# MayDomine/Burst-Attention

Measured on AMD Instinct MI355X. Metric: attention_fwd_TFLOPs_per_GPU, higher is better.
Workload: dtype fp16; 1 GPU; b=1 seq=262144 h=32 d=128 non-causal; parallelism=ring sequence parallel, sp1

## Files before the change

### burst_attn_amd/build_ext.py

```python

import os
import subprocess
import sys
import sysconfig

PKG_DIR = os.path.dirname(os.path.abspath(__file__))
CSRC = os.path.join(PKG_DIR, "csrc")
BUILD = os.path.join(PKG_DIR, "csrc", "_build")
ARCH = os.environ.get("PYTORCH_ROCM_ARCH", "gfx950")
HIPCC = os.environ.get("HIPCC", "/opt/rocm/bin/hipcc")

DEVICE_SOURCES = ["attn_fwd.hip", "attn_bwd.hip", "probes.hip"]
HOST_SOURCES = ["ext_torch.cpp"]


def _run(cmd, verbose):
    if verbose:
        print("+ " + " ".join(cmd), flush=True)
    r = subprocess.run(cmd, capture_output=True, text=True)
    if r.returncode != 0:
        sys.stderr.write(r.stdout + r.stderr)
        raise RuntimeError(f"build command failed: {' '.join(cmd[:3])} ...")
    return r


def _newer(src, dst):
    return not os.path.exists(dst) or os.path.getmtime(src) > os.path.getmtime(dst)


def build(verbose=True, force=False):
    import torch
    from torch.utils import cpp_extension

    os.makedirs(BUILD, exist_ok=True)
    out_so = os.path.join(PKG_DIR, "_C.so")

    torch_includes = cpp_extension.include_paths()
    py_include = sysconfig.get_paths()["include"]
    abi = int(torch._C._GLIBCXX_USE_CXX11_ABI)

    common = [
        f"--offload-arch={ARCH}", "-O3", "-std=c++17", "-fPIC",
        "-DNDEBUG",
    ]
    objs = []
    abihdr = os.path.join(PKG_DIR, "..", "include", "burst_attn_hip.h")
    hdrs = [abihdr] + [os.path.join(CSRC, h) for h in sorted(os.listdir(CSRC))
                       if h.endswith(".h")]
    for src in DEVICE_SOURCES:
        sp = os.path.join(CSRC, src)
        op = os.path.join(BUILD, src.replace(".hip", ".o"))
        objs.append(op)
        if force or _newer(sp, op) or any(_newer(h, op) for h in hdrs):
            _run([HIPCC, *common, "-c", sp, "-o", op], verbose)
    for src in HOST_SOURCES:
        sp = os.path.join(CSRC, src)
        op = os.path.join(BUILD, src.replace(".cpp", ".o"))
        objs.append(op)
        if force or _newer(sp, op) or any(_newer(h, op) for h in hdrs):
            cmd = [
                HIPCC, *common,
                f"-D_GLIBCXX_USE_CXX11_ABI={abi}",
                "-DTORCH_EXTENSION_NAME=_C",
                "-DTORCH_API_INCLUDE_EXTENSION_H",
                "-DUSE_ROCM=1", "-D__HIP_PLATFORM_AMD__=1",
            ]
            for inc in torch_includes + [py_include]:
                cmd += ["-I", inc]
            cmd += ["-c", sp, "-o", op]
            _run(cmd, verbose)
    if force or any(_newer(o, out_so) for o in objs):
        lib_dirs = cpp_extension.library_paths()
        cmd = [HIPCC, "-shared", "-fPIC", *objs, "-o", out_so]
        for ld in lib_dirs:
            cmd += [f"-L{ld}", f"-Wl,-rpath,{ld}"]
        cmd += ["-ltorch", "-ltorch_cpu", "-ltorch_python", "-lc10",
                "-ltorch_hip", "-lc10_hip", "-lamdhip64"]
        _run(cmd, verbose)
    _build_asm_hsaco(verbose, force)
    if verbose:
        print(f"built {out_so}")
    return out_so


LLVM = os.path.join(os.path.dirname(os.path.dirname(HIPCC)), "lib", "llvm",
                    "bin") if "rocm" in HIPCC else "/opt/rocm/lib/llvm/bin"


def _build_asm_hsaco(verbose, force):
    import json
    import re

    src = os.path.join(CSRC, "attn_fwd.hip")
    s_path = os.path.join(BUILD, "attn_fwd_scaffold.s")
    o_path = os.path.join(BUILD, "attn_fwd_scaffold.o")
    hsaco = os.path.join(PKG_DIR, "_asm_fwd.hsaco")
    syms = os.path.join(PKG_DIR, "_asm_fwd_syms.json")
    patch_mod = os.path.join(PKG_DIR, "..", "tools", "s_patch.py")
    if not (force or _newer(src, hsaco) or _newer(patch_mod, hsaco)):
        return hsaco
    _run([HIPCC, f"--offload-arch={ARCH}", "-O3", "-std=c++17", "-DNDEBUG",
          "-S", "--cuda-device-only", src, "-o", s_path], verbose)
    clang = os.path.join(LLVM, "clang")
    lld = os.path.join(LLVM, "ld.lld")
    _run([clang, "-x", "assembler", "-target", "amdgcn-amd-amdhsa",
          f"-mcpu={ARCH}", "-c", s_path, "-o", o_path], verbose)
    _run([lld, "-shared", o_path, "-o", hsaco], verbose)
    text = open(s_path).read()
    names = {}
    for key, pat in (
        ("f16_accum", r"_ZN12_GLOBAL__N_115attn_fwd_kernelIDF16_Li128ELi64ELi1ELi0ELi1ELi512ELi2ELi0ELi0EJEE\S*"),
        ("bf16_accum", r"_ZN12_GLOBAL__N_115attn_fwd_kernelIDF16bLi128ELi64ELi1ELi0ELi1ELi512ELi2ELi0ELi0EJEE\S*"),
    ):
        m = re.search(r"\.globl\t(" + pat + ")", text)
        if m:
            names[key] = m.group(1)
    with open(syms, "w") as f:
        json.dump(names, f, indent=1)
    import importlib.util

    spec = importlib.util.spec_from_file_location("s_patch", patch_mod)
    s_patch = importlib.util.module_from_spec(spec)
    spec.loader.exec_module(s_patch)
    sp_path = os.path.join(BUILD, "attn_fwd_patched.s")
    spo_path = os.path.join(BUILD, "attn_fwd_patched.o")
    hsaco_p = os.path.join(PKG_DIR, "_asm_fwd_p.hsaco")
    s_patch.apply("qk_split", s_path, sp_path, list(names.values()))
    _run([clang, "-x", "assembler", "-target", "amdgcn-amd-amdhsa",
          f"-mcpu={ARCH}", "-c", sp_path, "-o", spo_path], verbose)
    _run([lld, "-shared", spo_path, "-o", hsaco_p], verbose)
    if verbose:
        print(f"built {hsaco} and {hsaco_p} (qk_split)")
    return hsaco


if __name__ == "__main__":
    build(force="--force" in sys.argv)
```

### burst_attn_amd/csrc/attn_common.h

```cpp
#pragma once
#include <hip/hip_runtime.h>
#include <stdint.h>

#include "band_support.h"

typedef __attribute__((ext_vector_type(8))) __bf16 bf16x8_t;
typedef __attribute__((ext_vector_type(8))) _Float16 f16x8_t;
typedef __attribute__((ext_vector_type(16))) float f32x16_t;
typedef __attribute__((ext_vector_type(2))) int i32x2_t;
typedef __attribute__((ext_vector_type(4))) unsigned int u32x4_t;

__device__ __forceinline__ float ba_exp2(float x) {
  return __builtin_amdgcn_exp2f(x);
}

#define BA_LOG2E 1.44269504088896340736f
#define BA_LN2 0.69314718055994530942f
#define BA_NEG_BIG (-1e30f)

template <typename T>
struct mfma_traits;

template <>
struct mfma_traits<_Float16> {
  using frag = f16x8_t;
  static __device__ __forceinline__ f32x16_t mma(frag a, frag b, f32x16_t c) {
    return __builtin_amdgcn_mfma_f32_32x32x16_f16(a, b, c, 0, 0, 0);
  }
  static __device__ __forceinline__ unsigned int bits(float x) {
    _Float16 h = (_Float16)x;
    return (unsigned int)__builtin_bit_cast(unsigned short, h);
  }
  static __device__ __forceinline__ unsigned int pack2(float lo, float hi) {
    return __builtin_bit_cast(unsigned int, __builtin_amdgcn_cvt_pkrtz(lo, hi));
  }
};

template <>
struct mfma_traits<__bf16> {
  using frag = bf16x8_t;
  static __device__ __forceinline__ f32x16_t mma(frag a, frag b, f32x16_t c) {
    return __builtin_amdgcn_mfma_f32_32x32x16_bf16(a, b, c, 0, 0, 0);
  }
  static __device__ __forceinline__ unsigned int bits(float x) {
    __bf16 h = (__bf16)x;
    return (unsigned int)__builtin_bit_cast(unsigned short, h);
  }
  static __device__ __forceinline__ unsigned int pack2(float lo, float hi) {
    return bits(lo) | (bits(hi) << 16);
  }
};

__device__ __forceinline__ constexpr int ba_crow(int r, int hi) {
  return (r & 3) + 8 * (r >> 2) + 4 * hi;
}

template <int SWZ, int SWZ2 = 0>
__device__ __forceinline__ int ba_swz(int byte, int row) {
  return byte ^ ((((row & SWZ) ^ ((row >> 3) & SWZ2))) << 4);
}

template <typename T>
__device__ __forceinline__ void ba_build_frag_pair(
    const f32x16_t& p, typename mfma_traits<T>::frag out[2]) {
  using MT = mfma_traits<T>;
#pragma unroll
  for (int u = 0; u < 2; ++u) {
    unsigned int a0 = MT::pack2(p[8 * u + 0], p[8 * u + 1]);
    unsigned int a1 = MT::pack2(p[8 * u + 2], p[8 * u + 3]);
    unsigned int b0 = MT::pack2(p[8 * u + 4], p[8 * u + 5]);
    unsigned int b1 = MT::pack2(p[8 * u + 6], p[8 * u + 7]);
    i32x2_t r0 = __builtin_amdgcn_permlane32_swap((int)a0, (int)b0, false, false);
    i32x2_t r1 = __builtin_amdgcn_permlane32_swap((int)a1, (int)b1, false, false);
    u32x4_t w = {(unsigned int)r0[0], (unsigned int)r1[0],
                 (unsigned int)r0[1], (unsigned int)r1[1]};
    out[u] = __builtin_bit_cast(typename mfma_traits<T>::frag, w);
  }
}

__device__ __forceinline__ void ba_half_pair(float x, float& lo, float& hi) {
  const int xi = __builtin_bit_cast(int, x);
  const i32x2_t r = __builtin_amdgcn_permlane32_swap(xi, xi, false, false);
  lo = __builtin_bit_cast(float, (int)r[0]);
  hi = __builtin_bit_cast(float, (int)r[1]);
}

struct ba_seg_args {
  const int32_t* q_seg;
  const int32_t* kv_seg;
  int64_t q_sb, kv_sb;
  const int2* tile_mm;
  const int2* blk_range;
};
__device__ __forceinline__ ba_seg_args ba_seg_of() { return {}; }
__device__ __forceinline__ ba_seg_args ba_seg_of(const ba_seg_args& s) {
  return s;
}

template <typename A, typename B>
struct ba_same_t {
  static constexpr bool value = false;
};
template <typename A>
struct ba_same_t<A, A> {
  static constexpr bool value = true;
};
template <typename A, typename... P>
constexpr bool ba_pack_is = sizeof...(P) == 1 && (ba_same_t<A, P>::value && ...);
__device__ __forceinline__ ba_band_args ba_band_of(const ba_band_args& b) {
  return b;
}

__device__ __forceinline__ void ba_wave_minmax(int x, int& mn, int& mx) {
  mn = mx = x;
#pragma unroll
  for (int o = 32; o; o >>= 1) {
    mn = min(mn, __shfl_xor(mn, o));
    mx = max(mx, __shfl_xor(mx, o));
  }
  mn = __builtin_amdgcn_readfirstlane(mn);
  mx = __builtin_amdgcn_readfirstlane(mx);
}

__device__ __forceinline__ float ba_max16(const f32x16_t& v) {
  float a = fmaxf(fmaxf(v[0], v[1]), v[2]);
  float b = fmaxf(fmaxf(v[3], v[4]), v[5]);
  float c = fmaxf(fmaxf(v[6], v[7]), v[8]);
  float d = fmaxf(fmaxf(v[9], v[10]), v[11]);
  float e = fmaxf(fmaxf(v[12], v[13]), v[14]);
  float f = fmaxf(fmaxf(a, b), v[15]);
  return fmaxf(fmaxf(fmaxf(c, d), e), f);
}

template <typename T, int RS, int SWZ, int SWZ2 = 0>
__device__ __forceinline__ typename mfma_traits<T>::frag ba_ld_rowslice(
    const T* lds, int row, int elem0) {
  int byte = ba_swz<SWZ, SWZ2>(row * (2 * RS) + 2 * elem0, row);
  u32x4_t wv = *(const u32x4_t*)((const char*)lds + byte);
  return __builtin_bit_cast(typename mfma_traits<T>::frag, wv);
}

template <typename T, int RS_T, int SWZ_T, int SWZ2_T = 7>
__device__ __forceinline__ void ba_st_transposed(T* lds, int src_row, int d0,
                                                 const u32x4_t& chunk) {
  const T* e = (const T*)&chunk;
#pragma unroll
  for (int j = 0; j < 8; ++j) {
    const int row = d0 + j;
    const int byte = ba_swz<SWZ_T, SWZ2_T>(row * (2 * RS_T) + 2 * src_row, row);
    *(T*)((char*)lds + byte) = e[j];
  }
}

typedef __attribute__((ext_vector_type(4))) short s16x4_t;
typedef __attribute__((ext_vector_type(2))) unsigned int u32x2_t;

template <typename T, int D>
__device__ __forceinline__ int ba_tr16_byte(int lane, int kv0, int dbase) {
  const int kvr = kv0 + 8 * (lane >> 5) + ((lane >> 2) & 3);
  const int e16 = kvr * D + dbase + 16 * ((lane >> 4) & 1) + 4 * (lane & 3);
  return (2 * e16) ^ ((kvr & 7) << 3);
}

template <typename T, int D>
__device__ __forceinline__ typename mfma_traits<T>::frag ba_ld_tr16_frag(
    const T* lds, int lane, int kv0, int dbase) {
  auto p0 = (__attribute__((address_space(3))) s16x4_t*)((
      __attribute__((address_space(3))) char*)(lds) +
      ba_tr16_byte<T, D>(lane, kv0, dbase));
  auto p1 = (__attribute__((address_space(3))) s16x4_t*)((
      __attribute__((address_space(3))) char*)(lds) +
      ba_tr16_byte<T, D>(lane, kv0 + 4, dbase));
  s16x4_t lo = __builtin_amdgcn_ds_read_tr16_b64_v4i16(p0);
  s16x4_t hi = __builtin_amdgcn_ds_read_tr16_b64_v4i16(p1);
  u32x2_t l2 = __builtin_bit_cast(u32x2_t, lo);
  u32x2_t h2 = __builtin_bit_cast(u32x2_t, hi);
  u32x4_t w = {l2[0], l2[1], h2[0], h2[1]};
  return __builtin_bit_cast(typename mfma_traits<T>::frag, w);
}

template <typename T, int D>
__device__ __forceinline__ void ba_st_tr16row(T* lds, int kv, int d0,
                                              const u32x4_t& chunk) {
  const int b0 = (2 * (kv * D + d0)) ^ ((kv & 7) << 3);
  const int b1 = (2 * (kv * D + d0 + 4)) ^ ((kv & 7) << 3);
  u32x2_t lohalf = {chunk.x, chunk.y};
  u32x2_t hihalf = {chunk.z, chunk.w};
  *(u32x2_t*)((char*)lds + b0) = lohalf;
  *(u32x2_t*)((char*)lds + b1) = hihalf;
}
```

### burst_attn_amd/csrc/attn_fwd.hip

```cpp

#include "attn_common.h"
#include "attn_host.h"
#include "fwd_variants.h"
#include "gqa_heads.h"
#include "seg_support.h"
#include "vt_image.h"

#include <stddef.h>

namespace {

template <int N>
struct ba_ic {
  static constexpr int value = N;
};
struct ba_dyn {
  int value;
};
template <int N>
__device__ __forceinline__ int ba_buf_of(ba_ic<N>) { return N; }
__device__ __forceinline__ int ba_buf_of(ba_dyn d) { return d.value; }

template <typename T, int D, int KVBLK, int OUT_STATE, int VPATH, int SUBT,
          int NT = 512, int NBUF = 2, int KREG = 0, int VSRC = 0,
          typename... SEG>
__global__ __launch_bounds__(NT) void attn_fwd_kernel(
    const T* __restrict__ q, const T* __restrict__ k, const T* __restrict__ v,
    float* __restrict__ o, float* __restrict__ lse,
    int Sq, int Sk, int N, int G,
    int64_t q_sb, int64_t q_ss, int64_t q_sh,
    int64_t k_sb, int64_t k_ss, int64_t k_sh,
    int64_t v_sb, int64_t v_ss, int64_t v_sh,
    float scale, int causal,
    float* __restrict__ st_acc, float* __restrict__ st_m,
    float* __restrict__ st_l,
    int64_t a_sb, int64_t a_ss, int64_t a_sh,
    int64_t ml_sb, int64_t ml_sh, int carry_in, SEG... seg) {
  using MT = mfma_traits<T>;
  using frag = typename MT::frag;
  constexpr bool HAS_BAND = ba_pack_is<ba_band_args, SEG...>;
  constexpr bool HAS_SEG = sizeof...(SEG) != 0 && !HAS_BAND;
  constexpr bool HAS_MASK = HAS_SEG || HAS_BAND;
  static_assert(!HAS_MASK || (sizeof...(SEG) == 1 && VPATH == 0 && SUBT == 1 &&
                              NT == 512 && NBUF == 2 && KREG == 0 && VSRC == 0),
                "segment ids / band: the default variant, V transposed "
                "in-kernel");
  static_assert(!HAS_BAND || (KVBLK == BA_BAND_TILE && NT / 2 == BA_BAND_BLOCK),
                "band: the tile sizes of band_support.h");
  if constexpr (HAS_BAND) causal = 0;
  constexpr int SWZ_K = (D == 128) ? 15 : 7;
  constexpr int SWZ_V = 7;
  constexpr int PT = (KVBLK * D / 8) / NT;
  constexpr int QROWS = NT / 2;
  constexpr bool HSWAP = VSRC == 1;
  static_assert(PT >= 1, "tile must fill at least one chunk per thread");

  static_assert(KREG != 1 || (SUBT == 1 && NBUF == 2 && VPATH == 0),
                "KREG=1 path: SUBT=1, NBUF=2, V^T image only");
  static_assert(KREG != 2 || (SUBT == 1 && NBUF == 4 && VPATH == 0),
                "KREG=2 path: SUBT=1, NBUF=4 (cross-barrier prefetch)");
  static_assert(VSRC == 0 || (VPATH == 0 && SUBT == 1 && KREG == 0 &&
                              KVBLK == BA_VT_KVBLK),
                "the V^T image source: b128-read V^T LDS image, SUBT=1");
  constexpr int IMGS_F = (KREG == 1) ? 1 : 2;
  __shared__ T lds[NBUF * IMGS_F * KVBLK * D];
  auto ldsK = [&](int buf) -> T* { return lds + buf * (IMGS_F * KVBLK * D); };
  auto ldsVT = [&](int buf) -> T* {
    return lds + buf * (IMGS_F * KVBLK * D) + (KREG == 1 ? 0 : KVBLK * D);
  };

  const int tid = threadIdx.x;
  const int lane = tid & 63;
  const int wave = tid >> 6;
  const int l31 = lane & 31;
  const int hi = lane >> 5;
  const int n = blockIdx.y;
  const int b = blockIdx.z;
  const int qb = blockIdx.x * QROWS + wave * 32;
  const int q_row = qb + l31;

  const T* qp = q + (int64_t)b * q_sb + (int64_t)n * q_sh;
  const int nkv = n / G;
  const T* kp = k + (int64_t)b * k_sb + (int64_t)nkv * k_sh;
  const T* vp = v + (int64_t)b * v_sb + (int64_t)nkv * v_sh;

  frag qf[D / 16];
#pragma unroll
  for (int s = 0; s < D / 16; ++s) {
    if (q_row < Sq) {
      const T* src = qp + (int64_t)q_row * q_ss + 16 * s + 8 * hi;
      qf[s] = __builtin_bit_cast(frag, *(const u32x4_t*)src);
    } else {
      u32x4_t z = {0, 0, 0, 0};
      qf[s] = __builtin_bit_cast(frag, z);
    }
  }

  const float c2 = scale * BA_LOG2E;
  float m2 = BA_NEG_BIG;
  float lsum = 0.f;
  f32x16_t ot[D / 32];
#pragma unroll
  for (int dt = 0; dt < D / 32; ++dt) ot[dt] = (f32x16_t)(0.f);
  if (OUT_STATE && carry_in && q_row < Sq) {
    m2 = st_m[b * ml_sb + n * ml_sh + q_row];
    lsum = st_l[b * ml_sb + n * ml_sh + q_row];
    const float* arow = st_acc + b * a_sb + (int64_t)q_row * a_ss + n * a_sh;
#pragma unroll
    for (int dt = 0; dt < D / 32; ++dt)
#pragma unroll
      for (int r = 0; r < 16; ++r) ot[dt][r] = arow[dt * 32 + ba_crow(r, hi)];
  }

  const int kv_limit =
      causal ? min(Sk, (int)(blockIdx.x + 1) * QROWS) : Sk;
  const int nt_shape = (kv_limit + KVBLK - 1) / KVBLK;
  int2 trange = {0, nt_shape};
  int qid = 0, wq_min = 0, wq_max = 0;
  const int32_t* kseg = nullptr;
  const int2* tmm = nullptr;
  bool seg_mask = false;
  if constexpr (HAS_SEG) {
    const ba_seg_args sg = ba_seg_of(seg...);
    const int2 r = sg.blk_range[(int64_t)b * gridDim.x + blockIdx.x];
    trange.x = r.x;
    trange.y = min(trange.y, r.y);
    if (trange.x >= trange.y) {
      if (q_row < Sq && !(OUT_STATE && carry_in)) {
        float* row = OUT_STATE
                         ? st_acc + b * a_sb + (int64_t)q_row * a_ss + n * a_sh
                         : o + (((int64_t)b * Sq + q_row) * N + n) * D;
#pragma unroll
        for (int dt = 0; dt < D / 32; ++dt)
#pragma unroll
          for (int r2 = 0; r2 < 16; ++r2) row[dt * 32 + ba_crow(r2, hi)] = 0.f;
        if (hi == 0) {
          if (OUT_STATE) {
            st_m[b * ml_sb + n * ml_sh + q_row] = BA_NEG_BIG;
            st_l[b * ml_sb + n * ml_sh + q_row] = 0.f;
          } else {
            lse[((int64_t)b * N + n) * Sq + q_row] = -__builtin_inff();
          }
        }
      }
      return;
    }
    qid = sg.q_seg[b * sg.q_sb + min(q_row, Sq - 1)];
    ba_wave_minmax(qid, wq_min, wq_max);
    kseg = sg.kv_seg + b * sg.kv_sb;
    tmm = sg.tile_mm + (int64_t)b * ((Sk + KVBLK - 1) / KVBLK);
  }
  ba_band_args bd = {0, 0};
  bool band_full = false;
  if constexpr (HAS_BAND) {
    bd = ba_band_of(seg...);
    const ba_tile_range r = ba_band_block_tiles(blockIdx.x, bd, Sq, Sk);
    trange.x = r.lo;
    trange.y = r.hi;
    if (trange.x >= trange.y) {
      if (q_row < Sq && !(OUT_STATE && carry_in)) {
        float* row = OUT_STATE
                         ? st_acc + b * a_sb + (int64_t)q_row * a_ss + n * a_sh
                         : o + (((int64_t)b * Sq + q_row) * N + n) * D;
#pragma unroll
        for (int dt = 0; dt < D / 32; ++dt)
#pragma unroll
          for (int r2 = 0; r2 < 16; ++r2) row[dt * 32 + ba_crow(r2, hi)] = 0.f;
        if (hi == 0) {
          if (OUT_STATE) {
            st_m[b * ml_sb + n * ml_sh + q_row] = BA_NEG_BIG;
            st_l[b * ml_sb + n * ml_sh + q_row] = 0.f;
          } else {
            lse[((int64_t)b * N + n) * Sq + q_row] = -__builtin_inff();
          }
        }
      }
      return;
    }
  }
  const int t_first = HAS_MASK ? trange.x : 0;
  const int nt = HAS_MASK ? trange.y : nt_shape;
  static_assert(SUBT != 2 || (NBUF == 4 && VPATH == 0),
                "the T15 pipeline needs NBUF=4 and the V^T image");
  static_assert(SUBT != 3 || (NBUF == 4 && VPATH == 0 && NT == 256),
                "SUBT=3: NT=256 (1 wave/SIMD), NBUF=4, V^T image");

#define BA_STEP __attribute__((always_inline))
  auto k_frag = [&](int buf, int kvs, int s) BA_STEP {
    return ba_ld_rowslice<T, D, SWZ_K>(ldsK(buf), kvs * 32 + l31,
                                       16 * s + 8 * hi);
  };
  auto load_kfrags = [&](int buf, int kvs, frag* kf) BA_STEP {
#pragma unroll
    for (int s = 0; s < D / 16; ++s) kf[s] = k_frag(buf, kvs, s);
  };
  auto load_next_kfrags = [&](int t, int kvs, frag* kf) BA_STEP {
    const int nt_t = (kvs == 0) ? t : t + 1;
    if (nt_t < nt) load_kfrags(nt_t % NBUF, kvs ^ 1, kf);
  };
  auto qk_regs = [&](const frag* kf) BA_STEP {
    f32x16_t s = (f32x16_t)(0.f);
#pragma unroll
    for (int i = 0; i < D / 16; ++i) s = MT::mma(kf[i], qf[i], s);
    return s;
  };
  auto qk_lds = [&](int buf, int kvs) BA_STEP {
    f32x16_t s = (f32x16_t)(0.f);
#pragma unroll
    for (int i = 0; i < D / 16; ++i)
      s = MT::mma(k_frag(buf, kvs, i), qf[i], s);
    return s;
  };
  auto mask_sub = [&](f32x16_t& s, int base, int off) BA_STEP {
#pragma unroll
    for (int r = 0; r < 16; ++r) {
      const int kv_g = base + off + ba_crow(r, 0) + 4 * hi;
      if (!(kv_g < Sk && (!causal || kv_g <= q_row))) s[r] = BA_NEG_BIG;
      if constexpr (HAS_SEG) {
        if (seg_mask && kseg[min(kv_g, Sk - 1)] != qid) s[r] = BA_NEG_BIG;
      }
      if constexpr (HAS_BAND) {
        if (!ba_band_visible(q_row, kv_g, bd)) s[r] = BA_NEG_BIG;
      }
    }
  };
  auto row_max2 = [&](const f32x16_t& s) BA_STEP {
    float tm = ba_max16(s);
    if (HSWAP) {
      float lo, hi2;
      ba_half_pair(tm, lo, hi2);
      tm = fmaxf(lo, hi2);
    } else {
      tm = fmaxf(tm, __shfl_xor(tm, 32));
    }
    return tm * c2;
  };
  constexpr float DEFER_THR = 8.f;
  auto rescale = [&](float tm) BA_STEP {
    if (!__all(tm - m2 <= DEFER_THR)) {
      const float mnew = fmaxf(m2, tm);
      const float alpha = ba_exp2(m2 - mnew);
      m2 = mnew;
      lsum *= alpha;
#pragma unroll
      for (int dt = 0; dt < D / 32; ++dt)
#pragma unroll
        for (int r = 0; r < 16; ++r) ot[dt][r] *= alpha;
    }
  };
  auto softmax_tail = [&](f32x16_t& s, float tm, frag* pf) BA_STEP {
    rescale(tm);
    float rowsum = 0.f;
    if (HAS_BAND && band_full) {
#pragma unroll
      for (int r = 0; r < 16; ++r) {
        s[r] = ba_exp2(__builtin_fmaf(s[r], c2, -m2));
        rowsum += s[r];
      }
    } else {
#pragma unroll
      for (int r = 0; r < 16; ++r) {
        if constexpr (HAS_MASK) {
          const bool masked = s[r] == BA_NEG_BIG;
          s[r] = masked ? 0.f : ba_exp2(__builtin_fmaf(s[r], c2, -m2));
        } else {
          s[r] = ba_exp2(__builtin_fmaf(s[r], c2, -m2));
        }
        rowsum += s[r];
      }
    }
    if (HSWAP) {
      float lo, hi2;
      ba_half_pair(rowsum, lo, hi2);
      rowsum = lo + hi2;
    } else {
      rowsum += __shfl_xor(rowsum, 32);
    }
    lsum += rowsum;
    ba_build_frag_pair<T>(s, pf);
  };
  auto v_frag = [&](int buf, int drow, int kvc) BA_STEP -> frag {
    if (VPATH == 0)
      return ba_ld_rowslice<T, KVBLK, SWZ_V, 7>(ldsVT(buf), drow, kvc + 8 * hi);
    return ba_ld_tr16_frag<T, D>(ldsVT(buf), lane, kvc, drow & ~31);
  };
  auto pv_regs = [&](const frag* vv, const frag* pf) BA_STEP {
#pragma unroll
    for (int dt = 0; dt < D / 32; ++dt)
#pragma unroll
      for (int u = 0; u < 2; ++u)
        ot[dt] = MT::mma(vv[dt * 2 + u], pf[u], ot[dt]);
  };
  struct chunk_rc {
    int row, col8;
  };
  auto stage_rc = [&](int c) BA_STEP {
    const int flat = tid + c * NT;
    return chunk_rc{flat / (D / 8), flat % (D / 8)};
  };
#undef BA_STEP

  f32x16_t stP;
  int p_kv0 = -1;
  int p_cur = 0;
  bool p_full = false;
  auto push_scores = [&](const f32x16_t& s, int kv0s, int buf, bool full) {
    stP = s;
    p_kv0 = kv0s;
    p_cur = buf;
    p_full = full;
  };
  auto finish_subtile = [&]() {
    if (!p_full) mask_sub(stP, p_kv0, 0);
    frag pf[2];
    softmax_tail(stP, row_max2(stP), pf);
    const int kvs_l = (p_kv0 / 32) & 1;
#pragma unroll
    for (int dt = 0; dt < D / 32; ++dt) {
      const int drow = dt * 32 + l31;
#pragma unroll
      for (int u = 0; u < 2; ++u)
        ot[dt] = MT::mma(v_frag(p_cur, drow, kvs_l * 32 + 16 * u), pf[u],
                         ot[dt]);
    }
  };

  frag pvf[2];
  frag kfP[SUBT == 3 ? D / 16 : 1];
  frag vvP[SUBT == 3 ? D / 16 : 1];
  int v_kv0 = -1;

  auto phase3 = [&](bool steady, int t, int kvs, int cur3, bool full) {
    const f32x16_t stQ = qk_regs(kfP);
    load_next_kfrags(t, kvs, kfP);
    float tm = BA_NEG_BIG;
    if (steady || p_kv0 >= 0) {
      if (!p_full) mask_sub(stP, p_kv0, 0);
      tm = row_max2(stP);
    }
    if (steady || v_kv0 >= 0) pv_regs(vvP, pvf);
    if (steady || p_kv0 >= 0) {
      softmax_tail(stP, tm, pvf);
      v_kv0 = p_kv0;
      const int kvs_l = (p_kv0 / 32) & 1;
#pragma unroll
      for (int dt = 0; dt < D / 32; ++dt)
#pragma unroll
        for (int u = 0; u < 2; ++u)
          vvP[dt * 2 + u] = v_frag(p_cur, dt * 32 + l31, kvs_l * 32 + 16 * u);
    }
    push_scores(stQ, t * KVBLK + kvs * 32, cur3, full);
  };

  uint32_t k_loff[PT], v_loff[PT];
#pragma unroll
  for (int c = 0; c < PT; ++c) {
    const auto [row, col8] = stage_rc(c);
    k_loff[c] = (uint32_t)((row * k_ss + col8 * 8) * (int64_t)sizeof(T));
    v_loff[c] = (uint32_t)((row * v_ss + col8 * 8) * (int64_t)sizeof(T));
  }
  const bool stage_lin =
      (int64_t)(KVBLK - 1) * k_ss * (int64_t)sizeof(T) + 16 <= 0xffffffffLL &&
      (VSRC == 1 ||
       (int64_t)(KVBLK - 1) * v_ss * (int64_t)sizeof(T) + 16 <= 0xffffffffLL);
  auto issue_loads = [&](int tile, u32x4_t* kreg, u32x4_t* vreg) {
    const int kv0 = tile * KVBLK;
    if (VSRC == 1) {
      const char* vb = (const char*)(vp + tile * ba_vt_block_elems(D));
#pragma unroll
      for (int c = 0; c < PT; ++c)
        vreg[c] = *(const u32x4_t*)(vb + (uint32_t)((tid + c * NT) * 16));
    }
    if (SUBT == 1 && stage_lin && kv0 + KVBLK <= Sk) {
      const char* kb = (const char*)(kp + (int64_t)kv0 * k_ss);
      const char* vb = (const char*)(vp + (int64_t)kv0 * v_ss);
#pragma unroll
      for (int c = 0; c < PT; ++c) {
        if (KREG != 1) kreg[c] = *(const u32x4_t*)(kb + k_loff[c]);
        if (VSRC == 0) vreg[c] = *(const u32x4_t*)(vb + v_loff[c]);
      }
      return;
    }
#pragma unroll
    for (int c = 0; c < PT; ++c) {
      const auto [row, col8] = stage_rc(c);
      const int kvg = kv0 + row;
      const int kvc = kvg < Sk ? kvg : (Sk - 1);
      if (KREG != 1)
        kreg[c] = *(const u32x4_t*)(kp + (int64_t)kvc * k_ss + col8 * 8);
      if (VSRC == 0)
        vreg[c] = *(const u32x4_t*)(vp + (int64_t)kvc * v_ss + col8 * 8);
    }
  };
  auto write_lds = [&](int buf, const u32x4_t* kreg, const u32x4_t* vreg) {
#pragma unroll
    for (int c = 0; c < PT; ++c) {
      const auto [row, col8] = stage_rc(c);
      if (KREG != 1) {
        const int byte = ba_swz<SWZ_K>(row * (2 * D) + col8 * 16, row);
        *(u32x4_t*)((char*)ldsK(buf) + byte) = kreg[c];
      }
      if (VSRC == 1) {
        const int flat = tid + c * NT;
        const int byte = ba_swz<SWZ_V, 7>(flat * 16, flat / (KVBLK / 8));
        *(u32x4_t*)((char*)ldsVT(buf) + byte) = vreg[c];
      } else if (VPATH == 0)
        ba_st_transposed<T, KVBLK, SWZ_V, 7>(ldsVT(buf), row, col8 * 8, vreg[c]);
      else
        ba_st_tr16row<T, D>(ldsVT(buf), row, col8 * 8, vreg[c]);
    }
  };
  auto load_k_sub = [&](int tile, int kvs, frag* dst) {
#pragma unroll
    for (int s = 0; s < D / 16; ++s) {
      const int kvg = tile * KVBLK + kvs * 32 + l31;
      const int kvc = kvg < Sk ? kvg : (Sk - 1);
      dst[s] = __builtin_bit_cast(
          frag, *(const u32x4_t*)(kp + (int64_t)kvc * k_ss + 16 * s + 8 * hi));
    }
  };

  frag kfr[KREG == 1 ? 2 : 1][D / 16];
  {
    u32x4_t kreg[PT], vreg[PT];
    issue_loads(t_first, kreg, vreg);
    write_lds(0, kreg, vreg);
    if (KREG == 1) {
      load_k_sub(0, 0, kfr[0]);
      load_k_sub(0, 1, kfr[KREG == 1 ? 1 : 0]);
    }
    if (NBUF == 4 && nt > 1) {
      issue_loads(1, kreg, vreg);
      write_lds(1, kreg, vreg);
    }
    __syncthreads();
    if (KREG == 2) load_kfrags(0, 0, kfr[0]);
    if (SUBT == 3) load_kfrags(0, 0, kfP);
  }
  if (NT == 512 && __builtin_amdgcn_readfirstlane(threadIdx.x) >= 256)
    __builtin_amdgcn_s_setprio(1);

  constexpr int AHEAD = NBUF == 4 ? 2 : 1;
  auto tile_body = [&](int t, auto curc) {
    const int cur = ba_buf_of(curc);
    const int kv0 = t * KVBLK;
    const bool has_next = (t + AHEAD) < nt;
    u32x4_t kreg[PT], vreg[PT];
    if (has_next) issue_loads(t + AHEAD, kreg, vreg);

    bool active, full;
    if constexpr (HAS_SEG) {
      const int2 mm = tmm[t];
      seg_mask = !(mm.x == mm.y && wq_min == wq_max && mm.x == wq_min);
      active = (!causal || (kv0 <= qb + 31)) && mm.y >= wq_min &&
               mm.x <= wq_max;
      full = (kv0 + KVBLK <= Sk) && (!causal || (kv0 + KVBLK - 1 <= qb)) &&
             !seg_mask;
    } else if constexpr (HAS_BAND) {
      active = ba_band_wave_active(qb, kv0, bd);
      full = (kv0 + KVBLK <= Sk) && ba_band_wave_inside(qb, kv0, bd);
      band_full = full;
    } else {
      active = !causal || (kv0 <= qb + 31);
    }
    if (active) {
      if constexpr (!HAS_MASK)
        full = (kv0 + KVBLK <= Sk) && (!causal || (kv0 + KVBLK - 1 <= qb));
      if (SUBT == 3) {
        [[clang::always_inline]] phase3(false, t, 0, cur, full);
        [[clang::always_inline]] phase3(false, t, 1, cur, full);
      } else if (SUBT == 2) {
#pragma unroll
        for (int kvs = 0; kvs < 2; ++kvs) {
          const f32x16_t stQ = qk_lds(cur, kvs);
          if (p_kv0 >= 0) [[clang::always_inline]] finish_subtile();
          push_scores(stQ, kv0 + kvs * 32, cur, full);
        }
      } else if (SUBT == 1) {
#pragma unroll
        for (int kvs = 0; kvs < 2; ++kvs) {
          frag* kres = kfr[KREG == 1 ? kvs : 0];
          f32x16_t st = KREG ? qk_regs(kres) : qk_lds(cur, kvs);
          if (KREG == 1 && has_next) load_k_sub(t + AHEAD, kvs, kres);
          if (KREG == 2) load_next_kfrags(t, kvs, kres);
          if (!full) mask_sub(st, kv0, kvs * 32);
          frag pf[2];
          softmax_tail(st, row_max2(st), pf);
#pragma unroll
          for (int dt = 0; dt < D / 32; ++dt) {
            const int drow = dt * 32 + l31;
#pragma unroll
            for (int u = 0; u < 2; ++u)
              ot[dt] = MT::mma(v_frag(cur, drow, kvs * 32 + 16 * u), pf[u],
                               ot[dt]);
          }
        }
      } else {
        f32x16_t st[2] = {(f32x16_t)(0.f), (f32x16_t)(0.f)};
#pragma unroll
        for (int s = 0; s < D / 16; ++s) {
          frag k0 = ba_ld_rowslice<T, D, SWZ_K>(ldsK(cur), l31, 16 * s + 8 * hi);
          frag k1 =
              ba_ld_rowslice<T, D, SWZ_K>(ldsK(cur), 32 + l31, 16 * s + 8 * hi);
          st[0] = MT::mma(k0, qf[s], st[0]);
          st[1] = MT::mma(k1, qf[s], st[1]);
        }
        const bool full0 =
            (kv0 + KVBLK <= Sk) && (!causal || (kv0 + KVBLK - 1 <= qb));
        if (full0) {
#pragma unroll
          for (int r = 0; r < 16; ++r) {
            st[0][r] *= c2;
            st[1][r] *= c2;
          }
        } else {
#pragma unroll
          for (int r = 0; r < 16; ++r) {
            const int kv_g0 = kv0 + ba_crow(r, 0) + 4 * hi;
            const int kv_g1 = kv_g0 + 32;
            st[0][r] = (kv_g0 < Sk && (!causal || kv_g0 <= q_row))
                           ? st[0][r] * c2
                           : BA_NEG_BIG;
            st[1][r] = (kv_g1 < Sk && (!causal || kv_g1 <= q_row))
                           ? st[1][r] * c2
                           : BA_NEG_BIG;
          }
        }
        float tm = BA_NEG_BIG;
#pragma unroll
        for (int r = 0; r < 16; ++r) tm = fmaxf(tm, fmaxf(st[0][r], st[1][r]));
        tm = fmaxf(tm, __shfl_xor(tm, 32));
        rescale(tm);
        float rowsum = 0.f;
#pragma unroll
        for (int r = 0; r < 16; ++r) {
          st[0][r] = ba_exp2(st[0][r] - m2);
          st[1][r] = ba_exp2(st[1][r] - m2);
          rowsum += st[0][r] + st[1][r];
        }
        rowsum += __shfl_xor(rowsum, 32);
        lsum += rowsum;

        frag pf[2][2];
#pragma unroll
        for (int j = 0; j < 2; ++j) ba_build_frag_pair<T>(st[j], pf[j]);
#pragma unroll
        for (int dt = 0; dt < D / 32; ++dt) {
          const int drow = dt * 32 + l31;
#pragma unroll
          for (int u = 0; u < 2; ++u) {
            const frag v0 = v_frag(cur, drow, 16 * u);
            const frag v1 = v_frag(cur, drow, 32 + 16 * u);
            ot[dt] = MT::mma(v0, pf[0][u], ot[dt]);
            ot[dt] = MT::mma(v1, pf[1][u], ot[dt]);
          }
        }
      }
    }

    if (has_next) write_lds((cur + AHEAD) % NBUF, kreg, vreg);
    if (SUBT == 2 || SUBT == 3 || KREG == 2 || NBUF == 2 || (t & 1) ||
        t + 1 >= nt)
      __syncthreads();
  };
  if constexpr (SUBT == 1) {
    asm volatile(".p2align 7");
    for (int tb = t_first; tb < nt; tb += NBUF) {
      [[clang::always_inline]] tile_body(tb, ba_ic<0>{});
      if (tb + 1 < nt) [[clang::always_inline]] tile_body(tb + 1, ba_ic<1 % NBUF>{});
      if (NBUF > 2) {
        if (tb + 2 < nt) [[clang::always_inline]] tile_body(tb + 2, ba_ic<2 % NBUF>{});
        if (tb + 3 < nt) [[clang::always_inline]] tile_body(tb + 3, ba_ic<3 % NBUF>{});
      }
    }
  } else {
    for (int t = 0; t < nt; ++t)
      [[clang::always_inline]] tile_body(t, ba_dyn{t % NBUF});
  }
  if (SUBT == 2 && p_kv0 >= 0) finish_subtile();
  if (SUBT == 3) {
    if (v_kv0 >= 0) pv_regs(vvP, pvf);
    if (p_kv0 >= 0) finish_subtile();
  }

  if (q_row < Sq) {
    if (OUT_STATE) {
      float* arow = st_acc + b * a_sb + (int64_t)q_row * a_ss + n * a_sh;
#pragma unroll
      for (int dt = 0; dt < D / 32; ++dt)
#pragma unroll
        for (int r = 0; r < 16; ++r)
          arow[dt * 32 + ba_crow(r, hi)] = ot[dt][r];
      if (hi == 0) {
        st_m[b * ml_sb + n * ml_sh + q_row] = m2;
        st_l[b * ml_sb + n * ml_sh + q_row] = lsum;
      }
    } else {
      float inv_l = 1.f / lsum;
      if constexpr (HAS_MASK) inv_l = lsum == 0.f ? 0.f : inv_l;
      float* orow = o + (((int64_t)b * Sq + q_row) * N + n) * D;
#pragma unroll
      for (int dt = 0; dt < D / 32; ++dt)
#pragma unroll
        for (int r = 0; r < 16; ++r)
          orow[dt * 32 + ba_crow(r, hi)] = ot[dt][r] * inv_l;
      if (hi == 0)
        lse[((int64_t)b * N + n) * Sq + q_row] = BA_LN2 * (m2 + log2f(lsum));
    }
  }
}

template <typename T, int D>
__global__ void attn_fwd_finalize_kernel(
    const float* __restrict__ acc, const float* __restrict__ m,
    const float* __restrict__ l, T* __restrict__ o, float* __restrict__ lse,
    int S, int N) {
  const int lane = threadIdx.x & 63;
  const int wave = threadIdx.x >> 6;
  constexpr int LPR = D / 16;
  const int rows_per_wave = 64 / LPR;
  const int row_in = wave * rows_per_wave + lane / LPR;
  const int sub = lane % LPR;
  const int s = blockIdx.x * 4 * rows_per_wave + row_in;
  const int n = blockIdx.y, b = blockIdx.z;
  if (s >= S) return;
  const float lv = l[((int64_t)b * N + n) * S + s];
  const float inv_l = lv > 0.f ? 1.f / lv : 0.f;
  const float* arow = acc + (((int64_t)b * S + s) * N + n) * D + sub * 16;
  T* orow = o + (((int64_t)b * S + s) * N + n) * D + sub * 16;
#pragma unroll
  for (int j = 0; j < 16; ++j) orow[j] = (T)(arow[j] * inv_l);
  if (sub == 0)
    lse[((int64_t)b * N + n) * S + s] =
        BA_LN2 * (m[((int64_t)b * N + n) * S + s] + log2f(lv));
}

template <int V>
__global__ __launch_bounds__(256) void attn_fwd_state_init_kernel(
    float* __restrict__ acc, float* __restrict__ m, float* __restrict__ l,
    int S, int N, int D, int64_t a_sb, int64_t a_ss, int64_t a_sh,
    int64_t ml_sb, int64_t ml_sh) {
  const int dv = D / V;
  const int64_t i = (int64_t)blockIdx.x * 256 + threadIdx.x;
  const int b = blockIdx.y;
  if (i >= (int64_t)S * N * dv) return;
  const int d = (int)(i % dv) * V;
  const int n = (int)((i / dv) % N);
  const int s = (int)(i / ((int64_t)dv * N));
  float* row = acc + b * a_sb + (int64_t)s * a_ss + n * a_sh + d;
  if (V == 4) {
    *(float4*)row = make_float4(0.f, 0.f, 0.f, 0.f);
  } else {
    row[0] = 0.f;
  }
  if (d == 0) {
    m[b * ml_sb + n * ml_sh + s] = BA_NEG_BIG;
    l[b * ml_sb + n * ml_sh + s] = 0.f;
  }
}

template <typename T, int D>
__global__ __launch_bounds__(256) void attn_vt_image_kernel(
    const T* __restrict__ v, T* __restrict__ img, int Sk, int Nk,
    int64_t v_sb, int64_t v_ss, int64_t v_sh, int64_t img_elems) {
  constexpr int KVBLK = BA_VT_KVBLK;
  constexpr int NT = 256;
  constexpr int PT = (KVBLK * D / 8) / NT;
  __shared__ T lds[KVBLK * D];
  const int tid = threadIdx.x;
  const int t = blockIdx.x, nkv = blockIdx.y, b = blockIdx.z;
  const T* vp = v + (int64_t)b * v_sb + (int64_t)nkv * v_sh;
#pragma unroll
  for (int c = 0; c < PT; ++c) {
    const int flat = tid + c * NT;
    const int row = flat / (D / 8), col8 = flat % (D / 8);
    const int kvg = t * KVBLK + row;
    u32x4_t chunk = {0, 0, 0, 0};
    if (kvg < Sk)
      chunk = *(const u32x4_t*)(vp + (int64_t)kvg * v_ss + col8 * 8);
    ba_st_transposed<T, KVBLK, 7, 7>(lds, row, col8 * 8, chunk);
  }
  __syncthreads();
  const int64_t blk = ba_vt_offset(Nk, Sk, D, b, nkv, (int64_t)t * KVBLK, 0);
#pragma unroll
  for (int c = 0; c < PT; ++c) {
    const int flat = tid + c * NT;
    const auto f = ba_ld_rowslice<T, KVBLK, 7, 7>(lds, flat / (KVBLK / 8),
                                                  (flat % (KVBLK / 8)) * 8);
    const int64_t e = blk + (int64_t)flat * 8;
    if (e + 8 <= img_elems) *(u32x4_t*)(img + e) = __builtin_bit_cast(u32x4_t, f);
  }
}

__global__ __launch_bounds__(256) void seg_tile_minmax_kernel(
    const int32_t* __restrict__ ids, int64_t sb, int S, int ntiles,
    int2* __restrict__ mm, int* __restrict__ nonmono) {
  const int lane = threadIdx.x & 63;
  const int t = blockIdx.x * 4 + (threadIdx.x >> 6), b = blockIdx.y;
  if (t >= ntiles) return;
  const int i = min(t * BA_SEG_TILE + lane, S - 1);
  const int32_t* row = ids + b * sb;
  const int id = row[i];
  if (__any(row[max(i - 1, 0)] > id) && lane == 0) atomicOr(nonmono + b, 1);
  int mn, mx;
  ba_wave_minmax(id, mn, mx);
  if (lane == 0) mm[(int64_t)b * ntiles + t] = make_int2(mn, mx);
}

__global__ __launch_bounds__(256) void seg_block_range_kernel(
    const int32_t* __restrict__ ids, int64_t sb, int S,
    const int2* __restrict__ mm, int ntiles, const int* __restrict__ nonmono,
    int2* __restrict__ range) {
  __shared__ int s_min, s_max, s_lo, s_hi;
  const int tid = threadIdx.x, b = blockIdx.y;
  if (tid == 0) {
    s_min = INT32_MAX;
    s_max = INT32_MIN;
    s_lo = ntiles;
    s_hi = 0;
  }
  __syncthreads();
  int mn, mx;
  ba_wave_minmax(ids[b * sb + min((int)blockIdx.x * BA_SEG_BLOCK + tid, S - 1)],
                 mn, mx);
  if ((tid & 63) == 0) {
    atomicMin(&s_min, mn);
    atomicMax(&s_max, mx);
  }
  __syncthreads();
  const int bmin = s_min, bmax = s_max;
  const int2* m = mm + (int64_t)b * ntiles;
  int2* out = range + (int64_t)b * gridDim.x + blockIdx.x;
  if (!nonmono[b]) {
    if (tid == 0) {
      int lo = 0, hi = ntiles;
      while (lo < hi) {
        const int mid = (lo + hi) / 2;
        if (m[mid].y >= bmin) hi = mid; else lo = mid + 1;
      }
      int lo2 = lo, hi2 = ntiles;
      while (lo2 < hi2) {
        const int mid = (lo2 + hi2) / 2;
        if (m[mid].x > bmax) hi2 = mid; else lo2 = mid + 1;
      }
      *out = make_int2(lo, lo2);
    }
    return;
  }
  for (int t = tid; t < ntiles; t += 256)
    if (m[t].y >= bmin && m[t].x <= bmax) {
      atomicMin(&s_lo, t);
      atomicMax(&s_hi, t + 1);
    }
  __syncthreads();
  if (tid == 0) *out = make_int2(s_lo, s_hi);
}

}

int ba_seg_prepass(const int32_t* own, int64_t own_sb, int64_t S_own,
                   const int32_t* str, int64_t str_sb, int64_t S_str,
                   int64_t B, int32_t* flags, int32_t* tile_mm,
                   int32_t* blk_range, hipStream_t stream) {
  const int nt = (int)ba_seg_tiles(S_str), nb = (int)ba_seg_blocks(S_own);
  hipError_t e = hipMemsetAsync(flags, 0, (size_t)B * sizeof(int32_t), stream);
  if (e != hipSuccess)
    return ba_fail((int)e, "segment pre-pass memset failed: %s",
                   hipGetErrorString(e));
  seg_tile_minmax_kernel<<<dim3((unsigned)((nt + 3) / 4), (unsigned)B), 256, 0,
                           stream>>>(str, str_sb, (int)S_str, nt,
                                     (int2*)tile_mm, flags);
  seg_block_range_kernel<<<dim3((unsigned)nb, (unsigned)B), 256, 0, stream>>>(
      own, own_sb, (int)S_own, (const int2*)tile_mm, nt, flags,
      (int2*)blk_range);
  return ba_launch_status();
}

extern "C" const char* bahip_last_error(void) { return ba_g_err; }

struct fwd_args {
  const void *q, *k, *v;
  float *o, *lse;
  int Sq, Sk, N, G;
  int64_t q_sb, q_ss, q_sh, k_sb, k_ss, k_sh, v_sb, v_ss, v_sh;
  float scale;
  int causal;
  float *st_acc, *st_m, *st_l;
  int64_t a_sb, a_ss, a_sh, ml_sb, ml_sh;
  int carry_in;
};

using production_kernel_t = decltype(&attn_fwd_kernel<
    _Float16, 128, 64, 1, BA_FWD_PRODUCTION.vpath, BA_FWD_PRODUCTION.subt,
    BA_FWD_PRODUCTION.nt, BA_FWD_PRODUCTION.nbuf, BA_FWD_PRODUCTION.kreg>);
static_assert(offsetof(fwd_args, carry_in) + sizeof(int) ==
                      kernarg_size<production_kernel_t>::value &&
                  sizeof(fwd_args) ==
                      (kernarg_size<production_kernel_t>::value + 7) / 8 * 8,
              "fwd_args must mirror attn_fwd_kernel's parameter list");

static dim3 fwd_grid(const fwd_args& a, int64_t B, int nt) {
  return dim3((unsigned)((a.Sq + nt / 2 - 1) / (nt / 2)), (unsigned)a.N,
              (unsigned)B);
}

template <typename T, int D, int OUT_STATE, int VPATH, int SUBT, int NT,
          int NBUF, int KREG, int VSRC = 0>
static void launch_fwd(const fwd_args& a, int64_t B, hipStream_t stream) {
  attn_fwd_kernel<T, D, 64, OUT_STATE, VPATH, SUBT, NT, NBUF, KREG, VSRC>
      <<<fwd_grid(a, B, NT), dim3(NT), 0, stream>>>(
          (const T*)a.q, (const T*)a.k, (const T*)a.v, a.o, a.lse, a.Sq, a.Sk,
          a.N, a.G, a.q_sb, a.q_ss, a.q_sh, a.k_sb, a.k_ss, a.k_sh, a.v_sb, a.v_ss,
          a.v_sh, a.scale, a.causal, a.st_acc, a.st_m, a.st_l, a.a_sb, a.a_ss,
          a.a_sh, a.ml_sb, a.ml_sh, a.carry_in);
}

struct fwd_seg_call {
  const int32_t *q_seg, *kv_seg;
  int64_t q_sb, kv_sb;
  void* ws;
  int64_t ws_bytes;
};

static int seg_ids_given(const void* q_seg, const void* kv_seg, int* given) {
  if ((q_seg == nullptr) != (kv_seg == nullptr))
    return ba_fail(BAHIP_ERR_SEGMENT_IDS,
                   "segment ids: q_seg and kv_seg must both be given or both "
                   "be null (%s is null)",
                   q_seg ? "kv_seg" : "q_seg");
  *given = q_seg != nullptr;
  return 0;
}

static int fwd_default_variant_only(const char* what) {
  ba_fwd_knobs kn;
  kn.vpath = ba_env_int(BA_FWD_KNOB_SPECS[0].env, kn.vpath);
  kn.subt = ba_env_int(BA_FWD_KNOB_SPECS[1].env, kn.subt);
  kn.nt = ba_env_int(BA_FWD_KNOB_SPECS[2].env, kn.nt);
  kn.nbuf = ba_env_int(BA_FWD_KNOB_SPECS[3].env, kn.nbuf);
  kn.kreg = ba_env_int(BA_FWD_KNOB_SPECS[4].env, kn.kreg);
  const ba_fwd_choice c = ba_fwd_select(kn);
  if (c.bad_knob)
    return ba_fail(BAHIP_ERR_BAD_KNOB, "%s=%d is not an accepted value",
                   c.bad_knob, c.bad_value);
  const ba_seg_verdict sv = ba_seg_fwd_support(kn);
  if (sv.knob)
    return ba_fail(BAHIP_ERR_UNSUPPORTED,
                   "%s=%d does not support %s (default forward variant only)",
// ... 483 lines not shown
```

Baseline: 969.4 TFLOP/s/GPU.

## Permute K rows so S accumulators pack directly into P fragments

Loads K fragments with a swapped-bit row permutation (l31p), so the QK^T accumulator rows already come out in the order the PV MFMA B-operand expects. This lets the code replace the permlane32_swap-based fragment build with a direct pack, and the mask row indexing is updated to match. The change also switches tile loads to buffer loads with resource descriptors, drops the zero-initialised rowsum add, and compiles the forward kernel with -fno-honor-nans. The risk is correctness if the permutation does not exactly match the MFMA layout, and buffer range clamping can affect edge tiles.

```diff
diff --git a/burst_attn_amd/build_ext.py b/burst_attn_amd/build_ext.py
--- a/burst_attn_amd/build_ext.py
+++ b/burst_attn_amd/build_ext.py
@@ -12,6 +12,7 @@
 
 DEVICE_SOURCES = ["attn_fwd.hip", "attn_bwd.hip", "probes.hip"]
 HOST_SOURCES = ["ext_torch.cpp"]
+EXTRA_FLAGS = {"attn_fwd.hip": ["-fno-honor-nans"]}
 
 
 def _run(cmd, verbose):
@@ -52,7 +53,8 @@
         op = os.path.join(BUILD, src.replace(".hip", ".o"))
         objs.append(op)
         if force or _newer(sp, op) or any(_newer(h, op) for h in hdrs):
-            _run([HIPCC, *common, "-c", sp, "-o", op], verbose)
+            _run([HIPCC, *common, *EXTRA_FLAGS.get(src, []), "-c", sp, "-o", op],
+                 verbose)
     for src in HOST_SOURCES:
         sp = os.path.join(CSRC, src)
         op = os.path.join(BUILD, src.replace(".cpp", ".o"))
@@ -100,7 +102,8 @@
     if not (force or _newer(src, hsaco) or _newer(patch_mod, hsaco)):
         return hsaco
     _run([HIPCC, f"--offload-arch={ARCH}", "-O3", "-std=c++17", "-DNDEBUG",
-          "-S", "--cuda-device-only", src, "-o", s_path], verbose)
+          *EXTRA_FLAGS["attn_fwd.hip"], "-S", "--cuda-device-only", src,
+          "-o", s_path], verbose)
     clang = os.path.join(LLVM, "clang")
     lld = os.path.join(LLVM, "ld.lld")
     _run([clang, "-x", "assembler", "-target", "amdgcn-amd-amdhsa",
diff --git a/burst_attn_amd/csrc/attn_common.h b/burst_attn_amd/csrc/attn_common.h
--- a/burst_attn_amd/csrc/attn_common.h
+++ b/burst_attn_amd/csrc/attn_common.h
@@ -3,6 +3,7 @@
 #include <stdint.h>
 
 #include "band_support.h"
+#include "frag_perm.h"
 
 typedef __attribute__((ext_vector_type(8))) __bf16 bf16x8_t;
 typedef __attribute__((ext_vector_type(8))) _Float16 f16x8_t;
@@ -74,6 +75,20 @@
     i32x2_t r1 = __builtin_amdgcn_permlane32_swap((int)a1, (int)b1, false, false);
     u32x4_t w = {(unsigned int)r0[0], (unsigned int)r1[0],
                  (unsigned int)r0[1], (unsigned int)r1[1]};
+    out[u] = __builtin_bit_cast(typename mfma_traits<T>::frag, w);
+  }
+}
+
+template <typename T>
+__device__ __forceinline__ void ba_pack_frag_pair(
+    const f32x16_t& p, typename mfma_traits<T>::frag out[2]) {
+  using MT = mfma_traits<T>;
+#pragma unroll
+  for (int u = 0; u < 2; ++u) {
+    u32x4_t w = {MT::pack2(p[8 * u + 0], p[8 * u + 1]),
+                 MT::pack2(p[8 * u + 2], p[8 * u + 3]),
+                 MT::pack2(p[8 * u + 4], p[8 * u + 5]),
+                 MT::pack2(p[8 * u + 6], p[8 * u + 7])};
     out[u] = __builtin_bit_cast(typename mfma_traits<T>::frag, w);
   }
 }
diff --git a/burst_attn_amd/csrc/attn_fwd.hip b/burst_attn_amd/csrc/attn_fwd.hip
--- a/burst_attn_amd/csrc/attn_fwd.hip
+++ b/burst_attn_amd/csrc/attn_fwd.hip
@@ -73,6 +73,7 @@
   const int lane = tid & 63;
   const int wave = tid >> 6;
   const int l31 = lane & 31;
+  const int l31p = ba_swap23(l31);
   const int hi = lane >> 5;
   const int n = blockIdx.y;
   const int b = blockIdx.z;
@@ -187,7 +188,7 @@
 
 #define BA_STEP __attribute__((always_inline))
   auto k_frag = [&](int buf, int kvs, int s) BA_STEP {
-    return ba_ld_rowslice<T, D, SWZ_K>(ldsK(buf), kvs * 32 + l31,
+    return ba_ld_rowslice<T, D, SWZ_K>(ldsK(buf), kvs * 32 + l31p,
                                        16 * s + 8 * hi);
   };
   auto load_kfrags = [&](int buf, int kvs, frag* kf) BA_STEP {
@@ -214,7 +215,7 @@
   auto mask_sub = [&](f32x16_t& s, int base, int off) BA_STEP {
 #pragma unroll
     for (int r = 0; r < 16; ++r) {
-      const int kv_g = base + off + ba_crow(r, 0) + 4 * hi;
+      const int kv_g = base + off + ba_prow(r, 0) + 8 * hi;
       if (!(kv_g < Sk && (!causal || kv_g <= q_row))) s[r] = BA_NEG_BIG;
       if constexpr (HAS_SEG) {
         if (seg_mask && kseg[min(kv_g, Sk - 1)] != qid) s[r] = BA_NEG_BIG;
@@ -250,12 +251,12 @@
   };
   auto softmax_tail = [&](f32x16_t& s, float tm, frag* pf) BA_STEP {
     rescale(tm);
-    float rowsum = 0.f;
+    float rowsum;
     if (HAS_BAND && band_full) {
 #pragma unroll
       for (int r = 0; r < 16; ++r) {
         s[r] = ba_exp2(__builtin_fmaf(s[r], c2, -m2));
-        rowsum += s[r];
+        rowsum = r == 0 ? s[r] : rowsum + s[r];
       }
     } else {
 #pragma unroll
@@ -266,7 +267,7 @@
         } else {
           s[r] = ba_exp2(__builtin_fmaf(s[r], c2, -m2));
         }
-        rowsum += s[r];
+        rowsum = r == 0 ? s[r] : rowsum + s[r];
       }
     }
     if (HSWAP) {
@@ -277,7 +278,7 @@
       rowsum += __shfl_xor(rowsum, 32);
     }
     lsum += rowsum;
-    ba_build_frag_pair<T>(s, pf);
+    ba_pack_frag_pair<T>(s, pf);
   };
   auto v_frag = [&](int buf, int drow, int kvc) BA_STEP -> frag {
     if (VPATH == 0)
@@ -363,21 +364,33 @@
       (int64_t)(KVBLK - 1) * k_ss * (int64_t)sizeof(T) + 16 <= 0xffffffffLL &&
       (VSRC == 1 ||
        (int64_t)(KVBLK - 1) * v_ss * (int64_t)sizeof(T) + 16 <= 0xffffffffLL);
+  auto tile_rsrc = [&](const void* base, int64_t bytes) {
+    return __builtin_amdgcn_make_buffer_rsrc(
+        const_cast<void*>(base), 0,
+        (uint32_t)(bytes < 0xffffffffLL ? bytes : 0xffffffffLL), 0x00020000);
+  };
+  auto tile_span = [&](int64_t ss) {
+    return ((KVBLK - 1) * ss + D) * (int64_t)sizeof(T);
+  };
   auto issue_loads = [&](int tile, u32x4_t* kreg, u32x4_t* vreg) {
     const int kv0 = tile * KVBLK;
     if (VSRC == 1) {
-      const char* vb = (const char*)(vp + tile * ba_vt_block_elems(D));
+      const auto vr = tile_rsrc(vp + tile * ba_vt_block_elems(D),
+                                ba_vt_block_elems(D) * (int64_t)sizeof(T));
 #pragma unroll
       for (int c = 0; c < PT; ++c)
-        vreg[c] = *(const u32x4_t*)(vb + (uint32_t)((tid + c * NT) * 16));
+        vreg[c] = __builtin_amdgcn_raw_buffer_load_b128(vr, tid * 16,
+                                                        c * NT * 16, 0);
     }
     if (SUBT == 1 && stage_lin && kv0 + KVBLK <= Sk) {
-      const char* kb = (const char*)(kp + (int64_t)kv0 * k_ss);
-      const char* vb = (const char*)(vp + (int64_t)kv0 * v_ss);
+      const auto kr = tile_rsrc(kp + (int64_t)kv0 * k_ss, tile_span(k_ss));
+      const auto vr = tile_rsrc(vp + (int64_t)kv0 * v_ss, tile_span(v_ss));
 #pragma unroll
       for (int c = 0; c < PT; ++c) {
-        if (KREG != 1) kreg[c] = *(const u32x4_t*)(kb + k_loff[c]);
-        if (VSRC == 0) vreg[c] = *(const u32x4_t*)(vb + v_loff[c]);
+        if (KREG != 1)
+          kreg[c] = __builtin_amdgcn_raw_buffer_load_b128(kr, k_loff[c], 0, 0);
+        if (VSRC == 0)
+          vreg[c] = __builtin_amdgcn_raw_buffer_load_b128(vr, v_loff[c], 0, 0);
       }
       return;
     }
@@ -413,7 +426,7 @@
   auto load_k_sub = [&](int tile, int kvs, frag* dst) {
 #pragma unroll
     for (int s = 0; s < D / 16; ++s) {
-      const int kvg = tile * KVBLK + kvs * 32 + l31;
+      const int kvg = tile * KVBLK + kvs * 32 + l31p;
       const int kvc = kvg < Sk ? kvg : (Sk - 1);
       dst[s] = __builtin_bit_cast(
           frag, *(const u32x4_t*)(kp + (int64_t)kvc * k_ss + 16 * s + 8 * hi));
@@ -499,9 +512,9 @@
         f32x16_t st[2] = {(f32x16_t)(0.f), (f32x16_t)(0.f)};
 #pragma unroll
         for (int s = 0; s < D / 16; ++s) {
-          frag k0 = ba_ld_rowslice<T, D, SWZ_K>(ldsK(cur), l31, 16 * s + 8 * hi);
+          frag k0 = ba_ld_rowslice<T, D, SWZ_K>(ldsK(cur), l31p, 16 * s + 8 * hi);
           frag k1 =
-              ba_ld_rowslice<T, D, SWZ_K>(ldsK(cur), 32 + l31, 16 * s + 8 * hi);
+              ba_ld_rowslice<T, D, SWZ_K>(ldsK(cur), 32 + l31p, 16 * s + 8 * hi);
           st[0] = MT::mma(k0, qf[s], st[0]);
           st[1] = MT::mma(k1, qf[s], st[1]);
         }
@@ -516,7 +529,7 @@
         } else {
 #pragma unroll
           for (int r = 0; r < 16; ++r) {
-            const int kv_g0 = kv0 + ba_crow(r, 0) + 4 * hi;
+            const int kv_g0 = kv0 + ba_prow(r, 0) + 8 * hi;
             const int kv_g1 = kv_g0 + 32;
             st[0][r] = (kv_g0 < Sk && (!causal || kv_g0 <= q_row))
                            ? st[0][r] * c2
@@ -531,19 +544,20 @@
         for (int r = 0; r < 16; ++r) tm = fmaxf(tm, fmaxf(st[0][r], st[1][r]));
         tm = fmaxf(tm, __shfl_xor(tm, 32));
         rescale(tm);
-        float rowsum = 0.f;
+        float rowsum;
 #pragma unroll
         for (int r = 0; r < 16; ++r) {
           st[0][r] = ba_exp2(st[0][r] - m2);
           st[1][r] = ba_exp2(st[1][r] - m2);
-          rowsum += st[0][r] + st[1][r];
+          const float pair = st[0][r] + st[1][r];
+          rowsum = r == 0 ? pair : rowsum + pair;
         }
         rowsum += __shfl_xor(rowsum, 32);
         lsum += rowsum;
 
         frag pf[2][2];
 #pragma unroll
-        for (int j = 0; j < 2; ++j) ba_build_frag_pair<T>(st[j], pf[j]);
+        for (int j = 0; j < 2; ++j) ba_pack_frag_pair<T>(st[j], pf[j]);
 #pragma unroll
         for (int dt = 0; dt < D / 32; ++dt) {
           const int drow = dt * 32 + l31;
diff --git a/burst_attn_amd/csrc/frag_perm.h b/burst_attn_amd/csrc/frag_perm.h
--- /dev/null
+++ b/burst_attn_amd/csrc/frag_perm.h
@@ -0,0 +1,15 @@
+#pragma once
+
+#if defined(__HIPCC__) || defined(__CUDACC__)
+#define BA_PERM_FN __host__ __device__ constexpr
+#else
+#define BA_PERM_FN constexpr
+#endif
+
+BA_PERM_FN int ba_swap23(int i) {
+  return (i & ~12) | ((i & 4) << 1) | ((i & 8) >> 1);
+}
+
+BA_PERM_FN int ba_prow(int r, int hi) {
+  return 16 * (r >> 3) + 8 * hi + (r & 7);
+}
```

Measured after the change: 977.8 TFLOP/s/GPU (median of 6 runs). Within noise of the previous version (+0.9%).
